# tensorboy/centerpose

Hardware: AMD Instinct MI355X
Metric: images/sec end-to-end (backbone+decode), DLA-34 512x512 (higher is better)
Workload: dtype f32

## Files before the change

### centerpose_amd/csrc/head_wino24.hip

```cpp
#include "igemm.h"

#define HW_THREADS 512
#define HW_PH 18
#define HW_PW 18
#define HW_PWP 20
#define HW_C 64
#define HW_CGS (HW_C / 4)
#define HW_CG (HW_PH * HW_PWP * 4)
#define HW_PATCH (HW_CGS * HW_CG)
#define HW_F4 (HW_PH * HW_PW * HW_CGS)
#define HW_SLOTS ((HW_F4 + HW_THREADS - 1) / HW_THREADS)
#define HW_LDR 36
#define HW_RED (16 * 32 * HW_LDR)
#define HW_LDM 36
#define HW_MID (256 * HW_LDM)
#define HW_SMEM_FLOATS (2 * HW_RED)
#define HW_SMEM_FLOATS_MM (HW_RED + HW_MID > HW_PATCH ? HW_RED + HW_MID : HW_PATCH)

typedef float hw_v2 __attribute__((ext_vector_type(2)));
typedef float hw_v4 __attribute__((ext_vector_type(4)));

struct HwHead {
    const float* w2;
    const float* b2;
    float* out2;
    int n2, ld2, act2;
};
struct HwGrid {
    int tilesX, tilesY;
    unsigned mTx, mTy;
};
__device__ __forceinline__ hw_v4 hw_lds4(const float* p) { return *reinterpret_cast<const hw_v4*>(p); }
__device__ __forceinline__ int hw_div(int n, int d, unsigned magic) { return d == 1 ? n : (int)__umulhi((unsigned)n, magic); }

__device__ __forceinline__ void hw_write_share(const f32x16 (&acc)[3], const int vh, const int P, float* wq)
{
#pragma unroll
    for (int j = 0; j < 4; ++j) {
        hw_v4 q[3];
#pragma unroll
        for (int nu = 0; nu < 3; ++nu) q[nu] = (hw_v4){acc[nu][4 * j], acc[nu][4 * j + 1], acc[nu][4 * j + 2], acc[nu][4 * j + 3]};
        hw_v4 c0, c1;
        if (vh == 0) {
            const hw_v4 s1 = q[1] + q[2], d1 = q[1] - q[2];
            c0 = P == 0 ? q[0] + s1 : s1;
            c1 = d1;
        } else {
            const hw_v4 s2 = q[0] + q[1], d2 = q[0] - q[1];
            c0 = P == 0 ? s2 : 4.f * s2;
            c1 = P == 0 ? 2.f * d2 : 8.f * d2 + q[2];
        }
        *reinterpret_cast<hw_v4*>(wq + 8 * j) = c0;
        *reinterpret_cast<hw_v4*>(wq + 32 * HW_LDR + 8 * j) = c1;
    }
}

template <int N2, int MM, bool STAG>
__global__ __launch_bounds__(HW_THREADS, 1) void head_wino24_kernel(const ConvArgs a, const HwGrid gd, const HwHead hd)
{
    static_assert(!(STAG && MM), "the second-MFMA-phase form has no staggered variant");
    extern __shared__ __attribute__((aligned(16))) float smem[];
    const int tid = threadIdx.x, lane = tid & 63, wv = __builtin_amdgcn_readfirstlane(tid >> 6);
    const int xi = wv & 3, vh = wv >> 2;
    const int h = lane >> 5, m = lane & 31;
    const int NTILES = (a.Cout + 31) >> 5;
    int t_ = ig_xcd_remap(blockIdx.x, gridDim.x), q_;
    q_ = hw_div(t_, gd.tilesX, gd.mTx); const int tx = t_ - q_ * gd.tilesX; t_ = q_;
    q_ = hw_div(t_, gd.tilesY, gd.mTy); const int ty = t_ - q_ * gd.tilesY;
    const int b = q_;
    const int y0 = ty * 16, x0 = tx * 16;
    const int ld = a.srcLd[0];
    const float* __restrict__ x = a.src[0];

    {
        float4 rg[HW_SLOTS];
        int lo[HW_SLOTS];
        bool ok[HW_SLOTS];
#pragma unroll
        for (int s = 0; s < HW_SLOTS; ++s) {
            const int idx = tid + s * HW_THREADS;
            const int pp = idx / HW_CGS, q = idx % HW_CGS;
            const int py = pp / HW_PW, px = pp - py * HW_PW;
            const int gy = y0 - 1 + py, gx = x0 - 1 + px;
            const bool inl = idx < HW_F4;
            ok[s] = inl && gy >= 0 && gy < a.H && gx >= 0 && gx < a.W;
            const int go = ok[s] ? ((b * a.H + gy) * a.W + gx) * ld + q * 4 : 0;
            lo[s] = inl ? ((q * HW_PH + py) * HW_PWP + (px ^ ((py >> 1) & 3))) * 4 : -1;
            rg[s] = ig_ldg4(x + go);
        }
#pragma unroll
        for (int s = 0; s < HW_SLOTS; ++s)
            if (lo[s] >= 0) {
                float4 v = rg[s];
                if (!ok[s]) v = make_float4(0.f, 0.f, 0.f, 0.f);
                *reinterpret_cast<float4*>(smem + lo[s]) = v;
            }
    }
    const float* up = a.w + ((size_t)xi * NTILES * (HW_C / 8)) * 1536 + (size_t)(3 * vh) * 256 + lane * 4;
    const int nlin = NTILES * (HW_C / 8);
    float4 bq[2][3];
#pragma unroll
    for (int nu = 0; nu < 3; ++nu) bq[0][nu] = ig_ldg4(up + nu * 256);
    __syncthreads();
    if constexpr (STAG) {
        if (vh == 1) __syncthreads();
    }

    const int rA = xi == 0 ? 0 : (xi == 2 ? 2 : 1);
    const int rB = xi == 2 ? 1 : (xi == 3 ? 3 : 2);
    const float sg1 = xi == 1 ? 1.f : -1.f;
    const hw_v2 sg = {sg1, sg1};
    const int tyy = m >> 2, txx = m & 3;
    const int sA = (tyy + (rA >> 1)) & 3, sB = (tyy + (rB >> 1)) & 3;
    const int baseA = ((2 * tyy + rA) * HW_PWP + 4 * txx) * 4 + h * HW_CG;
    const int baseB = ((2 * tyy + rB) * HW_PWP + 4 * txx) * 4 + h * HW_CG;
    int offA[4], offB[4];
#pragma unroll
    for (int jj = 0; jj < 4; ++jj) { offA[jj] = baseA + ((jj ^ sA) << 2); offB[jj] = baseB + ((jj ^ sB) << 2); }
    hw_v2 vl[HW_C / 8][3], vhh[HW_C / 8][3];
#pragma unroll
    for (int kc = 0; kc < HW_C / 8; ++kc) {
        const float* pc = smem + kc * 2 * HW_CG;
        hw_v2 tl[5], th[5];
        if (vh == 0) {
#pragma unroll
            for (int j = 0; j < 5; ++j) {
                const hw_v4 da = hw_lds4(pc + offA[j & 3] + (j >> 2) * 16), db = hw_lds4(pc + offB[j & 3] + (j >> 2) * 16);
                tl[j] = __builtin_elementwise_fma(sg, db.xy, da.xy);
                th[j] = __builtin_elementwise_fma(sg, db.zw, da.zw);
            }
        } else {
#pragma unroll
            for (int j = 0; j < 5; ++j) {
                const int jc = j + 1;
                const hw_v4 da = hw_lds4(pc + offA[jc & 3] + (jc >> 2) * 16), db = hw_lds4(pc + offB[jc & 3] + (jc >> 2) * 16);
                tl[j] = __builtin_elementwise_fma(sg, db.xy, da.xy);
                th[j] = __builtin_elementwise_fma(sg, db.zw, da.zw);
            }
        }
        const hw_v2 k4 = {4.f, 4.f}, kn4 = {-4.f, -4.f}, k2 = {2.f, 2.f}, kn2 = {-2.f, -2.f};
        if (vh == 0) {
            const hw_v2 al = __builtin_elementwise_fma(kn4, tl[2], tl[4]), ah = __builtin_elementwise_fma(kn4, th[2], th[4]);
            const hw_v2 bl = __builtin_elementwise_fma(kn4, tl[1], tl[3]), bh = __builtin_elementwise_fma(kn4, th[1], th[3]);
            vl[kc][0] = __builtin_elementwise_fma(k4, tl[0] - tl[2], tl[4] - tl[2]); vhh[kc][0] = __builtin_elementwise_fma(k4, th[0] - th[2], th[4] - th[2]);
            vl[kc][1] = al + bl; vhh[kc][1] = ah + bh;
            vl[kc][2] = al - bl; vhh[kc][2] = ah - bh;
        } else {
            const hw_v2 cl = tl[3] - tl[1], ch = th[3] - th[1];
            const hw_v2 fl = tl[2] - tl[0], fh = th[2] - th[0];
            vl[kc][0] = __builtin_elementwise_fma(k2, fl, cl); vhh[kc][0] = __builtin_elementwise_fma(k2, fh, ch);
            vl[kc][1] = __builtin_elementwise_fma(kn2, fl, cl); vhh[kc][1] = __builtin_elementwise_fma(kn2, fh, ch);
            vl[kc][2] = __builtin_elementwise_fma(kn4, fl, tl[4] - tl[2]); vhh[kc][2] = __builtin_elementwise_fma(kn4, fh, th[4] - th[2]);
        }
#pragma unroll
        for (int nu = 0; nu < 3; ++nu) asm volatile("" : "+v"(vl[kc][nu]), "+v"(vhh[kc][nu]));
        __builtin_amdgcn_sched_barrier(0);
    }
    if constexpr (STAG) {
        if (vh == 0) __syncthreads();
    } else {
        __syncthreads();
    }

    float acc2[2][2][N2 > 0 ? N2 : 1];
#pragma unroll
    for (int i = 0; i < 2; ++i)
#pragma unroll
        for (int k = 0; k < 2; ++k)
#pragma unroll
            for (int j = 0; j < (N2 > 0 ? N2 : 1); ++j) acc2[i][k][j] = 0.f;
    f32x16 acc2m;
#pragma unroll
    for (int r = 0; r < 16; ++r) acc2m[r] = 0.f;
    constexpr int J0 = MM ? 32 : 0;
    float* const mid = smem + HW_RED;
    const int n4 = tid & 7, bb = (tid >> 3) & 1, mi = tid >> 4;
    const int ity = mi >> 2, itx = mi & 3;
    const int itrd = (bb * 32 + mi) * HW_LDR + n4 * 4;
    const int wpo = (wv * 64 + m) * HW_LDR + 4 * h;

    int lin = 0;
    if constexpr (!MM) {
        hw_v4 sc = {0.f, 0.f, 0.f, 0.f}, sh = sc, w2r[N2];
#pragma unroll
        for (int j = 0; j < N2; ++j) w2r[j] = sc;
        hw_v4 rq[8];
        auto red_read = [&](int P) __attribute__((always_inline)) {
            int rbase = itrd + P * HW_RED;
            asm volatile("" : "+v"(rbase));
            const float* rp = smem + rbase;
#pragma unroll
            for (int w = 0; w < 8; ++w) rq[w] = hw_lds4(rp + w * 64 * HW_LDR);
        };
        auto red_sum = [&](int P) __attribute__((always_inline)) {
            const hw_v4 r0 = rq[0] + rq[4], r1 = rq[1] + rq[5], r2 = rq[2] + rq[6], r3 = rq[3] + rq[7];
            hw_v4 yv[2];
            yv[0] = (r0 + r1) + r2;
            yv[1] = (r1 - r2) - r3;
#pragma unroll
            for (int aa = 0; aa < 2; ++aa) {
                hw_v4 v = __builtin_elementwise_fma(yv[aa], sc, sh);
                v = (hw_v4){cp_relu(v.x), cp_relu(v.y), cp_relu(v.z), cp_relu(v.w)};
#pragma unroll
                for (int j = 0; j < N2; ++j) {
                    const hw_v4 w = w2r[j];
                    acc2[P][aa][j] = fmaf(v.w, w.w, fmaf(v.z, w.z, fmaf(v.y, w.y, fmaf(v.x, w.x, acc2[P][aa][j]))));
                }
            }
        };
        if constexpr (STAG) {
            auto chunk = [&](const int kc, f32x16 (&acc)[3], auto&& ride) __attribute__((always_inline)) {
                ++lin;
                const float* un = up + (size_t)(lin < nlin ? lin : nlin - 1) * 1536;
                __builtin_amdgcn_sched_barrier(0);
#pragma unroll
                for (int nu = 0; nu < 3; ++nu) {
                    if (nu == 1) {
#pragma unroll
                        for (int q = 0; q < 3; ++q) bq[(kc + 1) & 1][q] = ig_ldg4(un + q * 256);
                        __builtin_amdgcn_sched_barrier(0);
                    }
                    if (nu == 2) {
                        ride();
                        __builtin_amdgcn_sched_barrier(0);
                    }
                    const float4 bbv = bq[kc & 1][nu];
                    acc[nu] = __builtin_amdgcn_mfma_f32_32x32x2f32(bbv.x, vl[kc][nu].x, acc[nu], 0, 0, 0);
                    acc[nu] = __builtin_amdgcn_mfma_f32_32x32x2f32(bbv.y, vl[kc][nu].y, acc[nu], 0, 0, 0);
                    acc[nu] = __builtin_amdgcn_mfma_f32_32x32x2f32(bbv.z, vhh[kc][nu].x, acc[nu], 0, 0, 0);
                    acc[nu] = __builtin_amdgcn_mfma_f32_32x32x2f32(bbv.w, vhh[kc][nu].y, acc[nu], 0, 0, 0);
                }
                __builtin_amdgcn_sched_barrier(0);
            };
            auto tile_end = [&](const int nt, const f32x16 (&acc)[3], const bool barrier_first) __attribute__((always_inline)) {
                const int ncol = nt * 32 + n4 * 4;
                sc = *reinterpret_cast<const hw_v4*>(a.scale + ncol);
                sh = *reinterpret_cast<const hw_v4*>(a.shift + ncol);
#pragma unroll
                for (int j = 0; j < N2; ++j) w2r[j] = *reinterpret_cast<const hw_v4*>(hd.w2 + (size_t)j * hd.ld2 + ncol);
                if (barrier_first) __syncthreads();
#pragma unroll
                for (int P = 0; P < 2; ++P) {
                    int wbase = wpo + P * HW_RED;
                    asm volatile("" : "+v"(wbase));
                    hw_write_share(acc, vh, P, smem + wbase);
                }
            };
            const auto nothing = [] {};
            if (vh == 0) {
#pragma unroll 1
                for (int nt = 0; nt < NTILES; ++nt) {
                    const bool prev = nt > 0;
                    f32x16 acc[3];
#pragma unroll
                    for (int nu = 0; nu < 3; ++nu)
#pragma unroll
                        for (int r = 0; r < 16; ++r) acc[nu][r] = 0.f;
#pragma unroll
                    for (int kc = 0; kc < 5; ++kc) chunk(kc, acc, nothing);
                    __syncthreads();
                    chunk(5, acc, [&] { if (prev) red_read(0); });
                    chunk(6, acc, [&] { if (prev) { red_sum(0); red_read(1); } });
                    chunk(7, acc, [&] { if (prev) red_sum(1); });
                    tile_end(nt, acc, true);
                }
            } else {
#pragma unroll 1
                for (int nt = 0; nt < NTILES; ++nt) {
                    const bool prev = nt > 0;
                    f32x16 acc[3];
#pragma unroll
                    for (int nu = 0; nu < 3; ++nu)
#pragma unroll
                        for (int r = 0; r < 16; ++r) acc[nu][r] = 0.f;
                    __syncthreads();
                    chunk(0, acc, [&] { if (prev) red_read(0); });
                    chunk(1, acc, [&] { if (prev) red_sum(0); });
                    chunk(2, acc, [&] { if (prev) red_read(1); });
                    chunk(3, acc, [&] { if (prev) red_sum(1); });
                    __syncthreads();
#pragma unroll
                    for (int kc = 4; kc < 8; ++kc) chunk(kc, acc, nothing);
                    tile_end(nt, acc, false);
                }
            }
            __syncthreads();
        } else {
#pragma unroll 1
        for (int nt = 0; nt < NTILES; ++nt) {
            const bool prev = nt > 0;
            f32x16 acc[3];
#pragma unroll
            for (int nu = 0; nu < 3; ++nu)
#pragma unroll
                for (int r = 0; r < 16; ++r) acc[nu][r] = 0.f;
#pragma unroll
            for (int kc = 0; kc < HW_C / 8; ++kc) {
                ++lin;
                const float* un = up + (size_t)(lin < nlin ? lin : nlin - 1) * 1536;
                __builtin_amdgcn_sched_barrier(0);
#pragma unroll
                for (int nu = 0; nu < 3; ++nu) {
                    if (nu == 1) {
#pragma unroll
                        for (int q = 0; q < 3; ++q) bq[(kc + 1) & 1][q] = ig_ldg4(un + q * 256);
                        __builtin_amdgcn_sched_barrier(0);
                    }
                    if (nu == 2 && prev) {
                        if (kc == 0) red_read(0);
                        if (kc == 2) red_sum(0);
                        if (kc == 4) red_read(1);
                        if (kc == 6) red_sum(1);
                        __builtin_amdgcn_sched_barrier(0);
                    }
                    const float4 bbv = bq[kc & 1][nu];
                    acc[nu] = __builtin_amdgcn_mfma_f32_32x32x2f32(bbv.x, vl[kc][nu].x, acc[nu], 0, 0, 0);
                    acc[nu] = __builtin_amdgcn_mfma_f32_32x32x2f32(bbv.y, vl[kc][nu].y, acc[nu], 0, 0, 0);
                    acc[nu] = __builtin_amdgcn_mfma_f32_32x32x2f32(bbv.z, vhh[kc][nu].x, acc[nu], 0, 0, 0);
                    acc[nu] = __builtin_amdgcn_mfma_f32_32x32x2f32(bbv.w, vhh[kc][nu].y, acc[nu], 0, 0, 0);
                }
                __builtin_amdgcn_sched_barrier(0);
            }
            const int ncol = nt * 32 + n4 * 4;
            sc = *reinterpret_cast<const hw_v4*>(a.scale + ncol);
            sh = *reinterpret_cast<const hw_v4*>(a.shift + ncol);
#pragma unroll
            for (int j = 0; j < N2; ++j) w2r[j] = *reinterpret_cast<const hw_v4*>(hd.w2 + (size_t)j * hd.ld2 + ncol);
            if (prev) __syncthreads();
#pragma unroll
            for (int P = 0; P < 2; ++P) {
                int wbase = wpo + P * HW_RED;
                asm volatile("" : "+v"(wbase));
                float* wq = smem + wbase;
#pragma unroll
                for (int j = 0; j < 4; ++j) {
                    hw_v4 q[3];
#pragma unroll
                    for (int nu = 0; nu < 3; ++nu) q[nu] = (hw_v4){acc[nu][4 * j], acc[nu][4 * j + 1], acc[nu][4 * j + 2], acc[nu][4 * j + 3]};
                    hw_v4 c0, c1;
                    if (vh == 0) {
                        const hw_v4 s1 = q[1] + q[2], d1 = q[1] - q[2];
                        c0 = P == 0 ? q[0] + s1 : s1;
                        c1 = d1;
                    } else {
                        const hw_v4 s2 = q[0] + q[1], d2 = q[0] - q[1];
                        c0 = P == 0 ? s2 : 4.f * s2;
                        c1 = P == 0 ? 2.f * d2 : 8.f * d2 + q[2];
                    }
                    *reinterpret_cast<hw_v4*>(wq + 8 * j) = c0;
                    *reinterpret_cast<hw_v4*>(wq + 32 * HW_LDR + 8 * j) = c1;
                }
            }
            __syncthreads();
        }
        }
        red_read(0); red_sum(0);
        red_read(1); red_sum(1);
    } else {
#pragma unroll 1
    for (int nt = 0; nt < NTILES; ++nt) {
        f32x16 acc[3];
#pragma unroll
        for (int nu = 0; nu < 3; ++nu)
#pragma unroll
            for (int r = 0; r < 16; ++r) acc[nu][r] = 0.f;
#pragma unroll
        for (int kc = 0; kc < HW_C / 8; ++kc) {
            ++lin;
            const float* un = up + (size_t)(lin < nlin ? lin : nlin - 1) * 1536;
            __builtin_amdgcn_sched_barrier(0);
#pragma unroll
            for (int nu = 0; nu < 3; ++nu) {
                if (nu == 1) {
#pragma unroll
                    for (int q = 0; q < 3; ++q) bq[(kc + 1) & 1][q] = ig_ldg4(un + q * 256);
                    __builtin_amdgcn_sched_barrier(0);
                }
                const float4 bbv = bq[kc & 1][nu];
                acc[nu] = __builtin_amdgcn_mfma_f32_32x32x2f32(bbv.x, vl[kc][nu].x, acc[nu], 0, 0, 0);
                acc[nu] = __builtin_amdgcn_mfma_f32_32x32x2f32(bbv.y, vl[kc][nu].y, acc[nu], 0, 0, 0);
                acc[nu] = __builtin_amdgcn_mfma_f32_32x32x2f32(bbv.z, vhh[kc][nu].x, acc[nu], 0, 0, 0);
                acc[nu] = __builtin_amdgcn_mfma_f32_32x32x2f32(bbv.w, vhh[kc][nu].y, acc[nu], 0, 0, 0);
            }
            __builtin_amdgcn_sched_barrier(0);
        }

        const int ncol = nt * 32 + n4 * 4;
        const hw_v4 sc = *reinterpret_cast<const hw_v4*>(a.scale + ncol), sh = *reinterpret_cast<const hw_v4*>(a.shift + ncol);
        hw_v4 w2r[N2 > 0 ? N2 : 1];
#pragma unroll
        for (int j = 0; j < N2; ++j) w2r[j] = *reinterpret_cast<const hw_v4*>(hd.w2 + (size_t)(J0 + j) * hd.ld2 + ncol);
        hw_v4 w2f[MM ? 4 : 1];
#pragma unroll
        for (int P = 0; P < 2; ++P) {
            if (MM && P == 1) __syncthreads();
            int wbase = wpo + (MM ? 0 : P * HW_RED), rbase = itrd + (MM ? 0 : P * HW_RED);
            asm volatile("" : "+v"(wbase), "+v"(rbase));
            float* wq = smem + wbase;
#pragma unroll
            for (int j = 0; j < 4; ++j) {
                hw_v4 q[3];
#pragma unroll
                for (int nu = 0; nu < 3; ++nu) q[nu] = (hw_v4){acc[nu][4 * j], acc[nu][4 * j + 1], acc[nu][4 * j + 2], acc[nu][4 * j + 3]};
                hw_v4 c0, c1;
                if (vh == 0) {
                    const hw_v4 s1 = q[1] + q[2], d1 = q[1] - q[2];
                    c0 = P == 0 ? q[0] + s1 : s1;
                    c1 = d1;
                } else {
                    const hw_v4 s2 = q[0] + q[1], d2 = q[0] - q[1];
                    c0 = P == 0 ? s2 : 4.f * s2;
                    c1 = P == 0 ? 2.f * d2 : 8.f * d2 + q[2];
                }
                *reinterpret_cast<hw_v4*>(wq + 8 * j) = c0;
                *reinterpret_cast<hw_v4*>(wq + 32 * HW_LDR + 8 * j) = c1;
            }
            if constexpr (MM) {
                if (P == 1) {
                    const int nmm = hd.n2 < 32 ? hd.n2 : 32;
                    const bool live = m < nmm;
                    const float* wrow = hd.w2 + (size_t)(live ? m : nmm - 1) * hd.ld2 + nt * 32 + 4 * h;
#pragma unroll
                    for (int s4 = 0; s4 < 4; ++s4) {
                        const float4 t4 = ig_ldg4(wrow + 8 * s4);
                        w2f[s4] = live ? (hw_v4){t4.x, t4.y, t4.z, t4.w} : (hw_v4){0.f, 0.f, 0.f, 0.f};
                    }
                }
            }
            __syncthreads();
            const float* rp = smem + rbase;
            hw_v4 r0 = hw_lds4(rp) + hw_lds4(rp + 4 * 64 * HW_LDR);
            const hw_v4 r1 = hw_lds4(rp + 64 * HW_LDR) + hw_lds4(rp + 5 * 64 * HW_LDR);
            const hw_v4 r2 = hw_lds4(rp + 2 * 64 * HW_LDR) + hw_lds4(rp + 6 * 64 * HW_LDR);
            const hw_v4 r3 = hw_lds4(rp + 3 * 64 * HW_LDR) + hw_lds4(rp + 7 * 64 * HW_LDR);
            hw_v4 yv[2];
            yv[0] = (r0 + r1) + r2;
            yv[1] = (r1 - r2) - r3;
#pragma unroll
            for (int aa = 0; aa < 2; ++aa) {
                hw_v4 v = __builtin_elementwise_fma(yv[aa], sc, sh);
                v = (hw_v4){cp_relu(v.x), cp_relu(v.y), cp_relu(v.z), cp_relu(v.w)};
#pragma unroll
                for (int j = 0; j < N2; ++j) {
                    const hw_v4 w = w2r[j];
                    acc2[P][aa][j] = fmaf(v.w, w.w, fmaf(v.z, w.z, fmaf(v.y, w.y, fmaf(v.x, w.x, acc2[P][aa][j]))));
                }
                if constexpr (MM) {
                    *reinterpret_cast<hw_v4*>(mid + ((2 * ity + aa) * 16 + 4 * itx + 2 * P + bb) * HW_LDM + n4 * 4) = v;
                }
            }
        }
        if constexpr (MM) {
            __syncthreads();
            const float* mp = mid + (32 * wv + m) * HW_LDM + 4 * h;
            hw_v4 mf[4];
#pragma unroll
            for (int s4 = 0; s4 < 4; ++s4) mf[s4] = hw_lds4(mp + 8 * s4);
#pragma unroll
            for (int s4 = 0; s4 < 4; ++s4) {
                acc2m = __builtin_amdgcn_mfma_f32_32x32x2f32(w2f[s4].x, mf[s4].x, acc2m, 0, 0, 0);
                acc2m = __builtin_amdgcn_mfma_f32_32x32x2f32(w2f[s4].y, mf[s4].y, acc2m, 0, 0, 0);
                acc2m = __builtin_amdgcn_mfma_f32_32x32x2f32(w2f[s4].z, mf[s4].z, acc2m, 0, 0, 0);
                acc2m = __builtin_amdgcn_mfma_f32_32x32x2f32(w2f[s4].w, mf[s4].w, acc2m, 0, 0, 0);
            }
            __syncthreads();
        }
    }

    }
    const size_t HW = (size_t)a.H * a.W;
    if constexpr (MM) {
        const int p = 32 * wv + m, ox = x0 + (p & 15), oy = y0 + (p >> 4);
        const int nmm = hd.n2 < 32 ? hd.n2 : 32;
        if (ox < a.W && oy < a.H) {
#pragma unroll
            for (int r = 0; r < 16; ++r) {
                const int j = (r & 3) + 8 * (r >> 2) + 4 * h;
                if (j < nmm) hd.out2[((size_t)b * hd.n2 + j) * HW + (size_t)oy * a.W + ox] = cp_act(acc2m[r] + hd.b2[j], hd.act2);
            }
        }
    }
    if constexpr (N2 > 0) {
#pragma unroll
        for (int P = 0; P < 2; ++P) {
            const int ox = x0 + 4 * itx + 2 * P + bb, oy = y0 + 2 * ity;
#pragma unroll
            for (int aa = 0; aa < 2; ++aa)
#pragma unroll
                for (int j = 0; j < N2; ++j) {
                    float v = acc2[P][aa][j];
                    v += __shfl_xor(v, 1);
                    v += __shfl_xor(v, 2);
                    v += __shfl_xor(v, 4);
                    if ((tid & 7) == 0 && J0 + j < hd.n2 && ox < a.W && oy + aa < a.H)
                        hd.out2[((size_t)b * hd.n2 + J0 + j) * HW + (size_t)(oy + aa) * a.W + ox] = cp_act(v + hd.b2[J0 + j], hd.act2);
                }
        }
    }
}

static unsigned hw_magic(int d) { return d <= 1 ? 0u : (unsigned)(((1ull << 32) + (unsigned)d - 1) / (unsigned)d); }

template <int N2, int MM, bool STAG = false>
static int launch_head_wino24(const ConvArgs& a, hipStream_t s, const HwHead& hd)
{
    const int smem = (MM ? HW_SMEM_FLOATS_MM : HW_SMEM_FLOATS) * 4;
    static CpLdsGuard guard;
    {
        const hipError_t e = guard.ensure((const void*)head_wino24_kernel<N2, MM, STAG>, smem);
        if (e != hipSuccess) { cp_set_error("head_wino24: cannot reserve %d B LDS: %s", smem, hipGetErrorString(e)); return 2; }
    }
    HwGrid gd;
    gd.tilesX = cp_cdiv(a.W, 16); gd.tilesY = cp_cdiv(a.H, 16);
    gd.mTx = hw_magic(gd.tilesX); gd.mTy = hw_magic(gd.tilesY);
    const long long grid = (long long)a.B * gd.tilesX * gd.tilesY;
    const long long dmax = gd.tilesX > gd.tilesY ? gd.tilesX : gd.tilesY;
    if (grid * dmax >= (1ll << 32)) { cp_set_error("head_wino24: grid %lld too large", grid); return 1; }
    hipLaunchKernelGGL((head_wino24_kernel<N2, MM, STAG>), dim3((unsigned)grid), dim3(HW_THREADS), smem, s, a, gd, hd);
    cp_note_kernel("head_wino24_kernel<%d, %d>", N2, MM);
    return 0;
}

int cp_launch_head3x3_1x1_w24(const ConvArgs& a, const float* w2, const float* b2, float* out2, int n2, int ld2, int act2, hipStream_t s)
{
    const bool ok = a.nsrc == 1 && a.kh == 3 && a.kw == 3 && a.sy == 1 && a.sx == 1 && a.py == 1 && a.px == 1 && a.Ho == a.H &&
                    a.Wo == a.W && a.srcC[0] == 64 && a.srcLd[0] % 4 == 0 && a.Cout % 32 == 0 && a.act == CP_ACT_RELU && !a.res &&
                    n2 >= 1 && n2 <= 34 && ld2 % 4 == 0 && ld2 >= a.Cout &&
                    (((size_t)a.src[0] | (size_t)a.w | (size_t)w2 | (size_t)a.scale | (size_t)a.shift) & 15) == 0 &&
                    (long long)a.B * a.H * a.W * a.srcLd[0] < (1ll << 31);
    if (!ok) return -1;
    HwHead hd;
    hd.w2 = w2; hd.b2 = b2; hd.out2 = out2; hd.n2 = n2; hd.ld2 = ld2; hd.act2 = act2;
    const char* sw = getenv("CP_HEAD_STAGGER");
    const bool stag = !(sw && sw[0] == '0');
    if (n2 == 1) return stag ? launch_head_wino24<1, 0, true>(a, s, hd) : launch_head_wino24<1, 0>(a, s, hd);
    if (n2 == 2) return stag ? launch_head_wino24<2, 0, true>(a, s, hd) : launch_head_wino24<2, 0>(a, s, hd);
    if (n2 <= 32) return launch_head_wino24<0, 1>(a, s, hd);
    if (n2 == 33) return launch_head_wino24<1, 1>(a, s, hd);
    return launch_head_wino24<2, 1>(a, s, hd);
}
```

Measured before the change: 2232.

## Make head Winograd kernel persistent with next-tile patch prefetch overlapped with MFMA

The head 3x3+1x1 Winograd kernel becomes a persistent loop over tiles. Each block computes the next tile's coordinates and issues its global patch loads during the current tile's MFMA phase, so the input fetch for tile n+1 overlaps compute for tile n. The grid is capped at the CU count only when CP_HEAD_PERSIST or CP_HEAD_BLOCKS is set, and the default trait is false. By default the grid still equals the tile count, so each block runs one iteration of the new loop structure and keeps the extra register pressure.

```diff
diff --git a/centerpose_amd/csrc/head_wino24.hip b/centerpose_amd/csrc/head_wino24.hip
--- a/centerpose_amd/csrc/head_wino24.hip
+++ b/centerpose_amd/csrc/head_wino24.hip
@@ -27,11 +27,17 @@
     int n2, ld2, act2;
 };
 struct HwGrid {
-    int tilesX, tilesY;
+    int tilesX, tilesY, tiles;
     unsigned mTx, mTy;
 };
+template <bool V> struct HwFlag { static constexpr bool value = V; };
 __device__ __forceinline__ hw_v4 hw_lds4(const float* p) { return *reinterpret_cast<const hw_v4*>(p); }
 __device__ __forceinline__ int hw_div(int n, int d, unsigned magic) { return d == 1 ? n : (int)__umulhi((unsigned)n, magic); }
+
+template <int K> __device__ __forceinline__ float hw_xor_lane(float v)
+{
+    return __int_as_float(__builtin_amdgcn_ds_swizzle(__float_as_int(v), (K << 10) | 0x1f));
+}
 
 __device__ __forceinline__ void hw_write_share(const f32x16 (&acc)[3], const int vh, const int P, float* wq)
 {
@@ -62,178 +68,226 @@
     extern __shared__ __attribute__((aligned(16))) float smem[];
     const int tid = threadIdx.x, lane = tid & 63, wv = __builtin_amdgcn_readfirstlane(tid >> 6);
     const int xi = wv & 3, vh = wv >> 2;
-    const int h = lane >> 5, m = lane & 31;
     const int NTILES = (a.Cout + 31) >> 5;
-    int t_ = ig_xcd_remap(blockIdx.x, gridDim.x), q_;
-    q_ = hw_div(t_, gd.tilesX, gd.mTx); const int tx = t_ - q_ * gd.tilesX; t_ = q_;
-    q_ = hw_div(t_, gd.tilesY, gd.mTy); const int ty = t_ - q_ * gd.tilesY;
-    const int b = q_;
-    const int y0 = ty * 16, x0 = tx * 16;
     const int ld = a.srcLd[0];
     const float* __restrict__ x = a.src[0];
-
-    {
-        float4 rg[HW_SLOTS];
-        int lo[HW_SLOTS];
-        bool ok[HW_SLOTS];
+    const int tiles = gd.tiles;
+
+    auto tile_at = [&](const int vv, int& b_, int& y0_, int& x0_) __attribute__((always_inline)) {
+        int t_ = ig_xcd_remap(vv, tiles), q_;
+        q_ = hw_div(t_, gd.tilesX, gd.mTx); x0_ = (t_ - q_ * gd.tilesX) * 16; t_ = q_;
+        q_ = hw_div(t_, gd.tilesY, gd.mTy); y0_ = (t_ - q_ * gd.tilesY) * 16;
+        b_ = q_;
+    };
+    float4 rg[HW_SLOTS];
+    unsigned okm;
+    auto patch_issue = [&](const int b_, const int y0_, const int x0_) __attribute__((always_inline)) {
+        int t = tid;
+        asm volatile("" : "+v"(t));
+        const int q = t & (HW_CGS - 1), pp0 = t >> 4;
+        okm = 0u;
 #pragma unroll
         for (int s = 0; s < HW_SLOTS; ++s) {
-            const int idx = tid + s * HW_THREADS;
-            const int pp = idx / HW_CGS, q = idx % HW_CGS;
+            const int pp = pp0 + s * (HW_THREADS / HW_CGS);
             const int py = pp / HW_PW, px = pp - py * HW_PW;
-            const int gy = y0 - 1 + py, gx = x0 - 1 + px;
-            const bool inl = idx < HW_F4;
-            ok[s] = inl && gy >= 0 && gy < a.H && gx >= 0 && gx < a.W;
-            const int go = ok[s] ? ((b * a.H + gy) * a.W + gx) * ld + q * 4 : 0;
-            lo[s] = inl ? ((q * HW_PH + py) * HW_PWP + (px ^ ((py >> 1) & 3))) * 4 : -1;
+            const int gy = y0_ - 1 + py, gx = x0_ - 1 + px;
+            const bool inl = (s + 1) * HW_THREADS <= HW_F4 || t + s * HW_THREADS < HW_F4;
+            const bool ok = inl && gy >= 0 && gy < a.H && gx >= 0 && gx < a.W;
+            const int go = ok ? ((b_ * a.H + gy) * a.W + gx) * ld + q * 4 : 0;
+            okm |= ok ? (1u << s) : 0u;
             rg[s] = ig_ldg4(x + go);
         }
-#pragma unroll
-        for (int s = 0; s < HW_SLOTS; ++s)
-            if (lo[s] >= 0) {
+    };
+    auto patch_store = [&]() __attribute__((always_inline)) {
+        int t = tid;
+        asm volatile("" : "+v"(t));
+        const int q = t & (HW_CGS - 1), pp0 = t >> 4;
+#pragma unroll
+        for (int s = 0; s < HW_SLOTS; ++s) {
+            const int pp = pp0 + s * (HW_THREADS / HW_CGS);
+            const int py = pp / HW_PW, px = pp - py * HW_PW;
+            if ((s + 1) * HW_THREADS <= HW_F4 || t + s * HW_THREADS < HW_F4) {
                 float4 v = rg[s];
-                if (!ok[s]) v = make_float4(0.f, 0.f, 0.f, 0.f);
-                *reinterpret_cast<float4*>(smem + lo[s]) = v;
-            }
-    }
-    const float* up = a.w + ((size_t)xi * NTILES * (HW_C / 8)) * 1536 + (size_t)(3 * vh) * 256 + lane * 4;
+                if (!((okm >> s) & 1u)) v = make_float4(0.f, 0.f, 0.f, 0.f);
+                *reinterpret_cast<float4*>(smem + ((q * HW_PH + py) * HW_PWP + (px ^ ((py >> 1) & 3))) * 4) = v;
+            }
+        }
+    };
+
+    int v = blockIdx.x, b, y0, x0;
+    tile_at(v, b, y0, x0);
+    patch_issue(b, y0, x0);
+    const float* up = a.w + ((size_t)xi * NTILES * (HW_C / 8)) * 1536 + (size_t)(3 * vh) * 256;
     const int nlin = NTILES * (HW_C / 8);
     float4 bq[2][3];
 #pragma unroll
-    for (int nu = 0; nu < 3; ++nu) bq[0][nu] = ig_ldg4(up + nu * 256);
-    __syncthreads();
-    if constexpr (STAG) {
-        if (vh == 1) __syncthreads();
-    }
+    for (int nu = 0; nu < 3; ++nu) bq[0][nu] = ig_ldg4(up + nu * 256 + (unsigned)lane * 4);
+    int lin = 0;
 
     const int rA = xi == 0 ? 0 : (xi == 2 ? 2 : 1);
     const int rB = xi == 2 ? 1 : (xi == 3 ? 3 : 2);
-    const float sg1 = xi == 1 ? 1.f : -1.f;
-    const hw_v2 sg = {sg1, sg1};
-    const int tyy = m >> 2, txx = m & 3;
-    const int sA = (tyy + (rA >> 1)) & 3, sB = (tyy + (rB >> 1)) & 3;
-    const int baseA = ((2 * tyy + rA) * HW_PWP + 4 * txx) * 4 + h * HW_CG;
-    const int baseB = ((2 * tyy + rB) * HW_PWP + 4 * txx) * 4 + h * HW_CG;
-    int offA[4], offB[4];
-#pragma unroll
-    for (int jj = 0; jj < 4; ++jj) { offA[jj] = baseA + ((jj ^ sA) << 2); offB[jj] = baseB + ((jj ^ sB) << 2); }
-    hw_v2 vl[HW_C / 8][3], vhh[HW_C / 8][3];
-#pragma unroll
-    for (int kc = 0; kc < HW_C / 8; ++kc) {
-        const float* pc = smem + kc * 2 * HW_CG;
-        hw_v2 tl[5], th[5];
-        if (vh == 0) {
-#pragma unroll
-            for (int j = 0; j < 5; ++j) {
-                const hw_v4 da = hw_lds4(pc + offA[j & 3] + (j >> 2) * 16), db = hw_lds4(pc + offB[j & 3] + (j >> 2) * 16);
-                tl[j] = __builtin_elementwise_fma(sg, db.xy, da.xy);
-                th[j] = __builtin_elementwise_fma(sg, db.zw, da.zw);
-            }
-        } else {
-#pragma unroll
-            for (int j = 0; j < 5; ++j) {
-                const int jc = j + 1;
-                const hw_v4 da = hw_lds4(pc + offA[jc & 3] + (jc >> 2) * 16), db = hw_lds4(pc + offB[jc & 3] + (jc >> 2) * 16);
-                tl[j] = __builtin_elementwise_fma(sg, db.xy, da.xy);
-                th[j] = __builtin_elementwise_fma(sg, db.zw, da.zw);
-            }
-        }
-        const hw_v2 k4 = {4.f, 4.f}, kn4 = {-4.f, -4.f}, k2 = {2.f, 2.f}, kn2 = {-2.f, -2.f};
-        if (vh == 0) {
-            const hw_v2 al = __builtin_elementwise_fma(kn4, tl[2], tl[4]), ah = __builtin_elementwise_fma(kn4, th[2], th[4]);
-            const hw_v2 bl = __builtin_elementwise_fma(kn4, tl[1], tl[3]), bh = __builtin_elementwise_fma(kn4, th[1], th[3]);
-            vl[kc][0] = __builtin_elementwise_fma(k4, tl[0] - tl[2], tl[4] - tl[2]); vhh[kc][0] = __builtin_elementwise_fma(k4, th[0] - th[2], th[4] - th[2]);
-            vl[kc][1] = al + bl; vhh[kc][1] = ah + bh;
-            vl[kc][2] = al - bl; vhh[kc][2] = ah - bh;
-        } else {
-            const hw_v2 cl = tl[3] - tl[1], ch = th[3] - th[1];
-            const hw_v2 fl = tl[2] - tl[0], fh = th[2] - th[0];
-            vl[kc][0] = __builtin_elementwise_fma(k2, fl, cl); vhh[kc][0] = __builtin_elementwise_fma(k2, fh, ch);
-            vl[kc][1] = __builtin_elementwise_fma(kn2, fl, cl); vhh[kc][1] = __builtin_elementwise_fma(kn2, fh, ch);
-            vl[kc][2] = __builtin_elementwise_fma(kn4, fl, tl[4] - tl[2]); vhh[kc][2] = __builtin_elementwise_fma(kn4, fh, th[4] - th[2]);
-        }
-#pragma unroll
-        for (int nu = 0; nu < 3; ++nu) asm volatile("" : "+v"(vl[kc][nu]), "+v"(vhh[kc][nu]));
-        __builtin_amdgcn_sched_barrier(0);
-    }
-    if constexpr (STAG) {
-        if (vh == 0) __syncthreads();
-    } else {
-        __syncthreads();
-    }
-
-    float acc2[2][2][N2 > 0 ? N2 : 1];
-#pragma unroll
-    for (int i = 0; i < 2; ++i)
-#pragma unroll
-        for (int k = 0; k < 2; ++k)
-#pragma unroll
-            for (int j = 0; j < (N2 > 0 ? N2 : 1); ++j) acc2[i][k][j] = 0.f;
-    f32x16 acc2m;
-#pragma unroll
-    for (int r = 0; r < 16; ++r) acc2m[r] = 0.f;
     constexpr int J0 = MM ? 32 : 0;
     float* const mid = smem + HW_RED;
-    const int n4 = tid & 7, bb = (tid >> 3) & 1, mi = tid >> 4;
-    const int ity = mi >> 2, itx = mi & 3;
-    const int itrd = (bb * 32 + mi) * HW_LDR + n4 * 4;
-    const int wpo = (wv * 64 + m) * HW_LDR + 4 * h;
-
-    int lin = 0;
-    if constexpr (!MM) {
-        hw_v4 sc = {0.f, 0.f, 0.f, 0.f}, sh = sc, w2r[N2];
-#pragma unroll
-        for (int j = 0; j < N2; ++j) w2r[j] = sc;
-        hw_v4 rq[8];
-        auto red_read = [&](int P) __attribute__((always_inline)) {
-            int rbase = itrd + P * HW_RED;
-            asm volatile("" : "+v"(rbase));
-            const float* rp = smem + rbase;
-#pragma unroll
-            for (int w = 0; w < 8; ++w) rq[w] = hw_lds4(rp + w * 64 * HW_LDR);
+    const size_t HW = (size_t)a.H * a.W;
+    float b2r[N2 > 0 ? N2 : 1];
+#pragma unroll
+    for (int j = 0; j < N2; ++j) b2r[j] = *(const __attribute__((address_space(4))) float*)(hd.b2 + J0 + j);
+
+#pragma unroll 1
+    for (;;) {
+        const int vn = v + (int)gridDim.x;
+        const bool more = vn < tiles;
+        int nb, ny0, nx0;
+        tile_at(more ? vn : v, nb, ny0, nx0);
+
+        patch_store();
+        __syncthreads();
+        if constexpr (STAG) {
+            if (vh == 1) __syncthreads();
+        }
+
+        int lv = tid & 63;
+        float sg1 = xi == 1 ? 1.f : -1.f;
+        asm volatile("" : "+v"(lv), "+v"(sg1));
+        const hw_v2 sg = {sg1, sg1};
+        const int tyy = (lv & 31) >> 2, txx = lv & 3;
+        const int sA = (tyy + (rA >> 1)) & 3, sB = (tyy + (rB >> 1)) & 3;
+        const int baseA = ((2 * tyy + rA) * HW_PWP + 4 * txx) * 4 + (lv >> 5) * HW_CG;
+        const int baseB = ((2 * tyy + rB) * HW_PWP + 4 * txx) * 4 + (lv >> 5) * HW_CG;
+        int offA[4], offB[4];
+#pragma unroll
+        for (int jj = 0; jj < 4; ++jj) { offA[jj] = baseA + ((jj ^ sA) << 2); offB[jj] = baseB + ((jj ^ sB) << 2); }
+        hw_v2 vl[HW_C / 8][3], vhh[HW_C / 8][3];
+#pragma unroll
+        for (int kc = 0; kc < HW_C / 8; ++kc) {
+            const float* pc = smem + kc * 2 * HW_CG;
+            hw_v2 tl[5], th[5];
+            if (vh == 0) {
+#pragma unroll
+                for (int j = 0; j < 5; ++j) {
+                    const hw_v4 da = hw_lds4(pc + offA[j & 3] + (j >> 2) * 16), db = hw_lds4(pc + offB[j & 3] + (j >> 2) * 16);
+                    tl[j] = __builtin_elementwise_fma(sg, db.xy, da.xy);
+                    th[j] = __builtin_elementwise_fma(sg, db.zw, da.zw);
+                }
+            } else {
+#pragma unroll
+                for (int j = 0; j < 5; ++j) {
+                    const int jc = j + 1;
+                    const hw_v4 da = hw_lds4(pc + offA[jc & 3] + (jc >> 2) * 16), db = hw_lds4(pc + offB[jc & 3] + (jc >> 2) * 16);
+                    tl[j] = __builtin_elementwise_fma(sg, db.xy, da.xy);
+                    th[j] = __builtin_elementwise_fma(sg, db.zw, da.zw);
+                }
+            }
+            const hw_v2 k4 = {4.f, 4.f}, kn4 = {-4.f, -4.f}, k2 = {2.f, 2.f}, kn2 = {-2.f, -2.f};
+            if (vh == 0) {
+                const hw_v2 al = __builtin_elementwise_fma(kn4, tl[2], tl[4]), ah = __builtin_elementwise_fma(kn4, th[2], th[4]);
+                const hw_v2 bl = __builtin_elementwise_fma(kn4, tl[1], tl[3]), bh = __builtin_elementwise_fma(kn4, th[1], th[3]);
+                vl[kc][0] = __builtin_elementwise_fma(k4, tl[0] - tl[2], tl[4] - tl[2]); vhh[kc][0] = __builtin_elementwise_fma(k4, th[0] - th[2], th[4] - th[2]);
+                vl[kc][1] = al + bl; vhh[kc][1] = ah + bh;
+                vl[kc][2] = al - bl; vhh[kc][2] = ah - bh;
+            } else {
+                const hw_v2 cl = tl[3] - tl[1], ch = th[3] - th[1];
+                const hw_v2 fl = tl[2] - tl[0], fh = th[2] - th[0];
+                vl[kc][0] = __builtin_elementwise_fma(k2, fl, cl); vhh[kc][0] = __builtin_elementwise_fma(k2, fh, ch);
+                vl[kc][1] = __builtin_elementwise_fma(kn2, fl, cl); vhh[kc][1] = __builtin_elementwise_fma(kn2, fh, ch);
+                vl[kc][2] = __builtin_elementwise_fma(kn4, fl, tl[4] - tl[2]); vhh[kc][2] = __builtin_elementwise_fma(kn4, fh, th[4] - th[2]);
+            }
+#pragma unroll
+            for (int nu = 0; nu < 3; ++nu) asm volatile("" : "+v"(vl[kc][nu]), "+v"(vhh[kc][nu]));
+            __builtin_amdgcn_sched_barrier(0);
+        }
+        if constexpr (STAG) {
+            if (vh == 0) __syncthreads();
+        } else {
+            __syncthreads();
+        }
+
+        float acc2[2][2][N2 > 0 ? N2 : 1];
+#pragma unroll
+        for (int i = 0; i < 2; ++i)
+#pragma unroll
+            for (int k = 0; k < 2; ++k)
+#pragma unroll
+                for (int j = 0; j < (N2 > 0 ? N2 : 1); ++j) acc2[i][k][j] = 0.f;
+        f32x16 acc2m;
+#pragma unroll
+        for (int r = 0; r < 16; ++r) acc2m[r] = 0.f;
+
+        auto chunk = [&](const int kc, f32x16 (&acc)[3], auto&& ride) __attribute__((always_inline)) {
+            lin = lin + 1 < nlin ? lin + 1 : 0;
+            const float* un = up + (size_t)lin * 1536;
+            int tc = tid;
+            asm volatile("" : "+v"(tc));
+            const unsigned ul = (tc & 63) * 4;
+            __builtin_amdgcn_sched_barrier(0);
+#pragma unroll
+            for (int nu = 0; nu < 3; ++nu) {
+                if (nu == 1) {
+#pragma unroll
+                    for (int q = 0; q < 3; ++q) bq[(kc + 1) & 1][q] = ig_ldg4(un + q * 256 + ul);
+                    __builtin_amdgcn_sched_barrier(0);
+                }
+                if (nu == 2) {
+                    ride();
+                    __builtin_amdgcn_sched_barrier(0);
+                }
+                const float4 bbv = bq[kc & 1][nu];
+                acc[nu] = __builtin_amdgcn_mfma_f32_32x32x2f32(bbv.x, vl[kc][nu].x, acc[nu], 0, 0, 0);
+                acc[nu] = __builtin_amdgcn_mfma_f32_32x32x2f32(bbv.y, vl[kc][nu].y, acc[nu], 0, 0, 0);
+                acc[nu] = __builtin_amdgcn_mfma_f32_32x32x2f32(bbv.z, vhh[kc][nu].x, acc[nu], 0, 0, 0);
+                acc[nu] = __builtin_amdgcn_mfma_f32_32x32x2f32(bbv.w, vhh[kc][nu].y, acc[nu], 0, 0, 0);
+            }
+            __builtin_amdgcn_sched_barrier(0);
         };
-        auto red_sum = [&](int P) __attribute__((always_inline)) {
-            const hw_v4 r0 = rq[0] + rq[4], r1 = rq[1] + rq[5], r2 = rq[2] + rq[6], r3 = rq[3] + rq[7];
-            hw_v4 yv[2];
-            yv[0] = (r0 + r1) + r2;
-            yv[1] = (r1 - r2) - r3;
-#pragma unroll
-            for (int aa = 0; aa < 2; ++aa) {
-                hw_v4 v = __builtin_elementwise_fma(yv[aa], sc, sh);
-                v = (hw_v4){cp_relu(v.x), cp_relu(v.y), cp_relu(v.z), cp_relu(v.w)};
-#pragma unroll
-                for (int j = 0; j < N2; ++j) {
-                    const hw_v4 w = w2r[j];
-                    acc2[P][aa][j] = fmaf(v.w, w.w, fmaf(v.z, w.z, fmaf(v.y, w.y, fmaf(v.x, w.x, acc2[P][aa][j]))));
-                }
-            }
+        auto request_next = [&]() __attribute__((always_inline)) {
+            if (more) {
+                patch_issue(nb, ny0, nx0);
+            } else {
+                okm = 0u;
+#pragma unroll
+                for (int s = 0; s < HW_SLOTS; ++s) rg[s] = make_float4(0.f, 0.f, 0.f, 0.f);
+            }
+            __builtin_amdgcn_sched_barrier(0);
         };
-        if constexpr (STAG) {
-            auto chunk = [&](const int kc, f32x16 (&acc)[3], auto&& ride) __attribute__((always_inline)) {
-                ++lin;
-                const float* un = up + (size_t)(lin < nlin ? lin : nlin - 1) * 1536;
-                __builtin_amdgcn_sched_barrier(0);
-#pragma unroll
-                for (int nu = 0; nu < 3; ++nu) {
-                    if (nu == 1) {
-#pragma unroll
-                        for (int q = 0; q < 3; ++q) bq[(kc + 1) & 1][q] = ig_ldg4(un + q * 256);
-                        __builtin_amdgcn_sched_barrier(0);
+        const auto nothing = [] {};
+
+        if constexpr (!MM) {
+            hw_v4 sc = {0.f, 0.f, 0.f, 0.f}, sh = sc, w2r[N2];
+#pragma unroll
+            for (int j = 0; j < N2; ++j) w2r[j] = sc;
+            hw_v4 rq[8];
+#pragma unroll
+            for (int w = 0; w < 8; ++w) rq[w] = sc;
+            auto red_read = [&](int P) __attribute__((always_inline)) {
+                int tr = tid;
+                asm volatile("" : "+v"(tr));
+                int rbase = (((tr >> 3) & 1) * 32 + (tr >> 4)) * HW_LDR + (tr & 7) * 4 + P * HW_RED;
+                asm volatile("" : "+v"(rbase));
+                const float* rp = smem + rbase;
+#pragma unroll
+                for (int w = 0; w < 8; ++w) rq[w] = hw_lds4(rp + w * 64 * HW_LDR);
+            };
+            auto red_sum = [&](int P) __attribute__((always_inline)) {
+                const hw_v4 r0 = rq[0] + rq[4], r1 = rq[1] + rq[5], r2 = rq[2] + rq[6], r3 = rq[3] + rq[7];
+                hw_v4 yv[2];
+                yv[0] = (r0 + r1) + r2;
+                yv[1] = (r1 - r2) - r3;
+#pragma unroll
+                for (int aa = 0; aa < 2; ++aa) {
+                    hw_v4 v = __builtin_elementwise_fma(yv[aa], sc, sh);
+                    v = (hw_v4){cp_relu(v.x), cp_relu(v.y), cp_relu(v.z), cp_relu(v.w)};
+#pragma unroll
+                    for (int j = 0; j < N2; ++j) {
+                        const hw_v4 w = w2r[j];
+                        acc2[P][aa][j] = fmaf(v.w, w.w, fmaf(v.z, w.z, fmaf(v.y, w.y, fmaf(v.x, w.x, acc2[P][aa][j]))));
                     }
-                    if (nu == 2) {
-                        ride();
-                        __builtin_amdgcn_sched_barrier(0);
-                    }
-                    const float4 bbv = bq[kc & 1][nu];
-                    acc[nu] = __builtin_amdgcn_mfma_f32_32x32x2f32(bbv.x, vl[kc][nu].x, acc[nu], 0, 0, 0);
-                    acc[nu] = __builtin_amdgcn_mfma_f32_32x32x2f32(bbv.y, vl[kc][nu].y, acc[nu], 0, 0, 0);
-                    acc[nu] = __builtin_amdgcn_mfma_f32_32x32x2f32(bbv.z, vhh[kc][nu].x, acc[nu], 0, 0, 0);
-                    acc[nu] = __builtin_amdgcn_mfma_f32_32x32x2f32(bbv.w, vhh[kc][nu].y, acc[nu], 0, 0, 0);
-                }
-                __builtin_amdgcn_sched_barrier(0);
+                }
             };
             auto tile_end = [&](const int nt, const f32x16 (&acc)[3], const bool barrier_first) __attribute__((always_inline)) {
-                const int ncol = nt * 32 + n4 * 4;
+                int nq = tid;
+                asm volatile("" : "+v"(nq));
+                nq &= 7;
+                const int ncol = nt * 32 + nq * 4;
                 sc = *reinterpret_cast<const hw_v4*>(a.scale + ncol);
                 sh = *reinterpret_cast<const hw_v4*>(a.shift + ncol);
 #pragma unroll
@@ -241,38 +295,37 @@
                 if (barrier_first) __syncthreads();
 #pragma unroll
                 for (int P = 0; P < 2; ++P) {
-                    int wbase = wpo + P * HW_RED;
+                    int tw = tid;
+                    asm volatile("" : "+v"(tw));
+                    int wbase = ((tw >> 6) * 64 + (tw & 31)) * HW_LDR + 4 * ((tw >> 5) & 1) + P * HW_RED;
                     asm volatile("" : "+v"(wbase));
                     hw_write_share(acc, vh, P, smem + wbase);
                 }
             };
-            const auto nothing = [] {};
-            if (vh == 0) {
-#pragma unroll 1
-                for (int nt = 0; nt < NTILES; ++nt) {
+            auto zero = [&](f32x16 (&acc)[3]) __attribute__((always_inline)) {
+#pragma unroll
+                for (int nu = 0; nu < 3; ++nu)
+#pragma unroll
+                    for (int r = 0; r < 16; ++r) acc[nu][r] = 0.f;
+            };
+            if constexpr (STAG) {
+                auto tileA = [&](const int nt, auto last) __attribute__((always_inline)) {
                     const bool prev = nt > 0;
                     f32x16 acc[3];
-#pragma unroll
-                    for (int nu = 0; nu < 3; ++nu)
-#pragma unroll
-                        for (int r = 0; r < 16; ++r) acc[nu][r] = 0.f;
+                    zero(acc);
 #pragma unroll
                     for (int kc = 0; kc < 5; ++kc) chunk(kc, acc, nothing);
                     __syncthreads();
                     chunk(5, acc, [&] { if (prev) red_read(0); });
                     chunk(6, acc, [&] { if (prev) { red_sum(0); red_read(1); } });
                     chunk(7, acc, [&] { if (prev) red_sum(1); });
+                    if constexpr (decltype(last)::value) request_next();
                     tile_end(nt, acc, true);
-                }
-            } else {
-#pragma unroll 1
-                for (int nt = 0; nt < NTILES; ++nt) {
+                };
+                auto tileB = [&](const int nt, auto last) __attribute__((always_inline)) {
                     const bool prev = nt > 0;
                     f32x16 acc[3];
-#pragma unroll
-                    for (int nu = 0; nu < 3; ++nu)
-#pragma unroll
-                        for (int r = 0; r < 16; ++r) acc[nu][r] = 0.f;
+                    zero(acc);
                     __syncthreads();
                     chunk(0, acc, [&] { if (prev) red_read(0); });
                     chunk(1, acc, [&] { if (prev) red_sum(0); });
@@ -281,225 +334,157 @@
                     __syncthreads();
 #pragma unroll
                     for (int kc = 4; kc < 8; ++kc) chunk(kc, acc, nothing);
+                    if constexpr (decltype(last)::value) request_next();
                     tile_end(nt, acc, false);
-                }
-            }
-            __syncthreads();
+                };
+                if (vh == 0) {
+#pragma unroll 1
+                    for (int nt = 0; nt < NTILES - 1; ++nt) tileA(nt, HwFlag<false>());
+                    tileA(NTILES - 1, HwFlag<true>());
+                } else {
+#pragma unroll 1
+                    for (int nt = 0; nt < NTILES - 1; ++nt) tileB(nt, HwFlag<false>());
+                    tileB(NTILES - 1, HwFlag<true>());
+                }
+                __syncthreads();
+            } else {
+                auto tileL = [&](const int nt, auto last) __attribute__((always_inline)) {
+                    const bool prev = nt > 0;
+                    f32x16 acc[3];
+                    zero(acc);
+                    chunk(0, acc, [&] { if (prev) red_read(0); });
+                    chunk(1, acc, nothing);
+                    chunk(2, acc, [&] { if (prev) red_sum(0); });
+                    chunk(3, acc, nothing);
+                    chunk(4, acc, [&] { if (prev) red_read(1); });
+                    chunk(5, acc, nothing);
+                    chunk(6, acc, [&] { if (prev) red_sum(1); });
+                    chunk(7, acc, nothing);
+                    if constexpr (decltype(last)::value) request_next();
+                    tile_end(nt, acc, prev);
+                    __syncthreads();
+                };
+#pragma unroll 1
+                for (int nt = 0; nt < NTILES - 1; ++nt) tileL(nt, HwFlag<false>());
+                tileL(NTILES - 1, HwFlag<true>());
+            }
+            red_read(0); red_sum(0);
+            red_read(1); red_sum(1);
         } else {
+            auto tileM = [&](const int nt, auto last) __attribute__((always_inline)) {
+                f32x16 acc[3];
+#pragma unroll
+                for (int nu = 0; nu < 3; ++nu)
+#pragma unroll
+                    for (int r = 0; r < 16; ++r) acc[nu][r] = 0.f;
+#pragma unroll
+                for (int kc = 0; kc < HW_C / 8; ++kc) chunk(kc, acc, nothing);
+                if constexpr (decltype(last)::value) request_next();
+
+                int te = tid;
+                asm volatile("" : "+v"(te));
+                const int nq = te & 7, eb = (te >> 3) & 1, emi = te >> 4, em = te & 31, eh = (te >> 5) & 1;
+                const int ncol = nt * 32 + nq * 4;
+                const hw_v4 sc = *reinterpret_cast<const hw_v4*>(a.scale + ncol), sh = *reinterpret_cast<const hw_v4*>(a.shift + ncol);
+                hw_v4 w2r[N2 > 0 ? N2 : 1];
+#pragma unroll
+                for (int j = 0; j < N2; ++j) w2r[j] = *reinterpret_cast<const hw_v4*>(hd.w2 + (size_t)(J0 + j) * hd.ld2 + ncol);
+                hw_v4 w2f[4];
+#pragma unroll
+                for (int P = 0; P < 2; ++P) {
+                    if (P == 1) __syncthreads();
+                    int wbase = ((te >> 6) * 64 + em) * HW_LDR + 4 * eh, rbase = (eb * 32 + emi) * HW_LDR + nq * 4;
+                    asm volatile("" : "+v"(wbase), "+v"(rbase));
+                    hw_write_share(acc, vh, P, smem + wbase);
+                    if (P == 1) {
+                        const int nmm = hd.n2 < 32 ? hd.n2 : 32;
+                        const bool live = em < nmm;
+                        const float* wrow = hd.w2 + (size_t)(live ? em : nmm - 1) * hd.ld2 + nt * 32 + 4 * eh;
+#pragma unroll
+                        for (int s4 = 0; s4 < 4; ++s4) {
+                            const float4 t4 = ig_ldg4(wrow + 8 * s4);
+                            w2f[s4] = live ? (hw_v4){t4.x, t4.y, t4.z, t4.w} : (hw_v4){0.f, 0.f, 0.f, 0.f};
+                        }
+                    }
+                    __syncthreads();
+                    const float* rp = smem + rbase;
+                    hw_v4 r0 = hw_lds4(rp) + hw_lds4(rp + 4 * 64 * HW_LDR);
+                    const hw_v4 r1 = hw_lds4(rp + 64 * HW_LDR) + hw_lds4(rp + 5 * 64 * HW_LDR);
+                    const hw_v4 r2 = hw_lds4(rp + 2 * 64 * HW_LDR) + hw_lds4(rp + 6 * 64 * HW_LDR);
+                    const hw_v4 r3 = hw_lds4(rp + 3 * 64 * HW_LDR) + hw_lds4(rp + 7 * 64 * HW_LDR);
+                    hw_v4 yv[2];
+                    yv[0] = (r0 + r1) + r2;
+                    yv[1] = (r1 - r2) - r3;
+#pragma unroll
+                    for (int aa = 0; aa < 2; ++aa) {
+                        hw_v4 v = __builtin_elementwise_fma(yv[aa], sc, sh);
+                        v = (hw_v4){cp_relu(v.x), cp_relu(v.y), cp_relu(v.z), cp_relu(v.w)};
+#pragma unroll
+                        for (int j = 0; j < N2; ++j) {
+                            const hw_v4 w = w2r[j];
+                            acc2[P][aa][j] = fmaf(v.w, w.w, fmaf(v.z, w.z, fmaf(v.y, w.y, fmaf(v.x, w.x, acc2[P][aa][j]))));
+                        }
+                        *reinterpret_cast<hw_v4*>(mid + ((2 * (emi >> 2) + aa) * 16 + 4 * (emi & 3) + 2 * P + eb) * HW_LDM + nq * 4) = v;
+                    }
+                }
+                __syncthreads();
+                const float* mp = mid + (32 * wv + em) * HW_LDM + 4 * eh;
+                hw_v4 mf[4];
+#pragma unroll
+                for (int s4 = 0; s4 < 4; ++s4) mf[s4] = hw_lds4(mp + 8 * s4);
+#pragma unroll
+                for (int s4 = 0; s4 < 4; ++s4) {
+                    acc2m = __builtin_amdgcn_mfma_f32_32x32x2f32(w2f[s4].x, mf[s4].x, acc2m, 0, 0, 0);
+                    acc2m = __builtin_amdgcn_mfma_f32_32x32x2f32(w2f[s4].y, mf[s4].y, acc2m, 0, 0, 0);
+                    acc2m = __builtin_amdgcn_mfma_f32_32x32x2f32(w2f[s4].z, mf[s4].z, acc2m, 0, 0, 0);
+                    acc2m = __builtin_amdgcn_mfma_f32_32x32x2f32(w2f[s4].w, mf[s4].w, acc2m, 0, 0, 0);
+                }
+                __syncthreads();
+            };
 #pragma unroll 1
-        for (int nt = 0; nt < NTILES; ++nt) {
-            const bool prev = nt > 0;
-            f32x16 acc[3];
-#pragma unroll
-            for (int nu = 0; nu < 3; ++nu)
-#pragma unroll
-                for (int r = 0; r < 16; ++r) acc[nu][r] = 0.f;
-#pragma unroll
-            for (int kc = 0; kc < HW_C / 8; ++kc) {
-                ++lin;
-                const float* un = up + (size_t)(lin < nlin ? lin : nlin - 1) * 1536;
-                __builtin_amdgcn_sched_barrier(0);
-#pragma unroll
-                for (int nu = 0; nu < 3; ++nu) {
-                    if (nu == 1) {
-#pragma unroll
-                        for (int q = 0; q < 3; ++q) bq[(kc + 1) & 1][q] = ig_ldg4(un + q * 256);
-                        __builtin_amdgcn_sched_barrier(0);
+            for (int nt = 0; nt < NTILES - 1; ++nt) tileM(nt, HwFlag<false>());
+            tileM(NTILES - 1, HwFlag<true>());
+        }
+
+        int to = tid;
+        asm volatile("" : "+v"(to));
+        if constexpr (MM) {
+            const int p = 32 * wv + (to & 31), ox = x0 + (p & 15), oy = y0 + (p >> 4);
+            const int nmm = hd.n2 < 32 ? hd.n2 : 32;
+            if (ox < a.W && oy < a.H) {
+#pragma unroll
+                for (int r = 0; r < 16; ++r) {
+                    const int j = (r & 3) + 8 * (r >> 2) + 4 * ((to >> 5) & 1);
+                    if (j < nmm) hd.out2[((size_t)b * hd.n2 + j) * HW + (size_t)oy * a.W + ox] = cp_act(acc2m[r] + hd.b2[j], hd.act2);
+                }
+            }
+        }
+        if constexpr (N2 > 0) {
+#pragma unroll
+            for (int P = 0; P < 2; ++P) {
+                const int ox = x0 + 4 * ((to >> 4) & 3) + 2 * P + ((to >> 3) & 1), oy = y0 + 2 * (to >> 6);
+#pragma unroll
+                for (int aa = 0; aa < 2; ++aa)
+#pragma unroll
+                    for (int j = 0; j < N2; ++j) {
+                        float v = acc2[P][aa][j];
+                        v += hw_xor_lane<1>(v);
+                        v += hw_xor_lane<2>(v);
+                        v += hw_xor_lane<4>(v);
+                        if ((to & 7) == 0 && J0 + j < hd.n2 && ox < a.W && oy + aa < a.H)
+                            hd.out2[((size_t)b * hd.n2 + J0 + j) * HW + (size_t)(oy + aa) * a.W + ox] = cp_act(v + b2r[j], hd.act2);
                     }
-                    if (nu == 2 && prev) {
-                        if (kc == 0) red_read(0);
-                        if (kc == 2) red_sum(0);
-                        if (kc == 4) red_read(1);
-                        if (kc == 6) red_sum(1);
-                        __builtin_amdgcn_sched_barrier(0);
-                    }
-                    const float4 bbv = bq[kc & 1][nu];
-                    acc[nu] = __builtin_amdgcn_mfma_f32_32x32x2f32(bbv.x, vl[kc][nu].x, acc[nu], 0, 0, 0);
-                    acc[nu] = __builtin_amdgcn_mfma_f32_32x32x2f32(bbv.y, vl[kc][nu].y, acc[nu], 0, 0, 0);
-                    acc[nu] = __builtin_amdgcn_mfma_f32_32x32x2f32(bbv.z, vhh[kc][nu].x, acc[nu], 0, 0, 0);
-                    acc[nu] = __builtin_amdgcn_mfma_f32_32x32x2f32(bbv.w, vhh[kc][nu].y, acc[nu], 0, 0, 0);
-                }
-                __builtin_amdgcn_sched_barrier(0);
-            }
-            const int ncol = nt * 32 + n4 * 4;
-            sc = *reinterpret_cast<const hw_v4*>(a.scale + ncol);
-            sh = *reinterpret_cast<const hw_v4*>(a.shift + ncol);
-#pragma unroll
-            for (int j = 0; j < N2; ++j) w2r[j] = *reinterpret_cast<const hw_v4*>(hd.w2 + (size_t)j * hd.ld2 + ncol);
-            if (prev) __syncthreads();
-#pragma unroll
-            for (int P = 0; P < 2; ++P) {
-                int wbase = wpo + P * HW_RED;
-                asm volatile("" : "+v"(wbase));
-                float* wq = smem + wbase;
-#pragma unroll
-                for (int j = 0; j < 4; ++j) {
-                    hw_v4 q[3];
-#pragma unroll
-                    for (int nu = 0; nu < 3; ++nu) q[nu] = (hw_v4){acc[nu][4 * j], acc[nu][4 * j + 1], acc[nu][4 * j + 2], acc[nu][4 * j + 3]};
-                    hw_v4 c0, c1;
-                    if (vh == 0) {
-                        const hw_v4 s1 = q[1] + q[2], d1 = q[1] - q[2];
-                        c0 = P == 0 ? q[0] + s1 : s1;
-                        c1 = d1;
-                    } else {
-                        const hw_v4 s2 = q[0] + q[1], d2 = q[0] - q[1];
-                        c0 = P == 0 ? s2 : 4.f * s2;
-                        c1 = P == 0 ? 2.f * d2 : 8.f * d2 + q[2];
-                    }
-                    *reinterpret_cast<hw_v4*>(wq + 8 * j) = c0;
-                    *reinterpret_cast<hw_v4*>(wq + 32 * HW_LDR + 8 * j) = c1;
-                }
-            }
-            __syncthreads();
-        }
-        }
-        red_read(0); red_sum(0);
-        red_read(1); red_sum(1);
-    } else {
-#pragma unroll 1
-    for (int nt = 0; nt < NTILES; ++nt) {
-        f32x16 acc[3];
-#pragma unroll
-        for (int nu = 0; nu < 3; ++nu)
-#pragma unroll
-            for (int r = 0; r < 16; ++r) acc[nu][r] = 0.f;
-#pragma unroll
-        for (int kc = 0; kc < HW_C / 8; ++kc) {
-            ++lin;
-            const float* un = up + (size_t)(lin < nlin ? lin : nlin - 1) * 1536;
-            __builtin_amdgcn_sched_barrier(0);
-#pragma unroll
-            for (int nu = 0; nu < 3; ++nu) {
-                if (nu == 1) {
-#pragma unroll
-                    for (int q = 0; q < 3; ++q) bq[(kc + 1) & 1][q] = ig_ldg4(un + q * 256);
-                    __builtin_amdgcn_sched_barrier(0);
-                }
-                const float4 bbv = bq[kc & 1][nu];
-                acc[nu] = __builtin_amdgcn_mfma_f32_32x32x2f32(bbv.x, vl[kc][nu].x, acc[nu], 0, 0, 0);
-                acc[nu] = __builtin_amdgcn_mfma_f32_32x32x2f32(bbv.y, vl[kc][nu].y, acc[nu], 0, 0, 0);
-                acc[nu] = __builtin_amdgcn_mfma_f32_32x32x2f32(bbv.z, vhh[kc][nu].x, acc[nu], 0, 0, 0);
-                acc[nu] = __builtin_amdgcn_mfma_f32_32x32x2f32(bbv.w, vhh[kc][nu].y, acc[nu], 0, 0, 0);
-            }
-            __builtin_amdgcn_sched_barrier(0);
-        }
-
-        const int ncol = nt * 32 + n4 * 4;
-        const hw_v4 sc = *reinterpret_cast<const hw_v4*>(a.scale + ncol), sh = *reinterpret_cast<const hw_v4*>(a.shift + ncol);
-        hw_v4 w2r[N2 > 0 ? N2 : 1];
-#pragma unroll
-        for (int j = 0; j < N2; ++j) w2r[j] = *reinterpret_cast<const hw_v4*>(hd.w2 + (size_t)(J0 + j) * hd.ld2 + ncol);
-        hw_v4 w2f[MM ? 4 : 1];
-#pragma unroll
-        for (int P = 0; P < 2; ++P) {
-            if (MM && P == 1) __syncthreads();
-            int wbase = wpo + (MM ? 0 : P * HW_RED), rbase = itrd + (MM ? 0 : P * HW_RED);
-            asm volatile("" : "+v"(wbase), "+v"(rbase));
-            float* wq = smem + wbase;
-#pragma unroll
-            for (int j = 0; j < 4; ++j) {
-                hw_v4 q[3];
-#pragma unroll
-                for (int nu = 0; nu < 3; ++nu) q[nu] = (hw_v4){acc[nu][4 * j], acc[nu][4 * j + 1], acc[nu][4 * j + 2], acc[nu][4 * j + 3]};
-                hw_v4 c0, c1;
-                if (vh == 0) {
-                    const hw_v4 s1 = q[1] + q[2], d1 = q[1] - q[2];
-                    c0 = P == 0 ? q[0] + s1 : s1;
-                    c1 = d1;
-                } else {
-                    const hw_v4 s2 = q[0] + q[1], d2 = q[0] - q[1];
-                    c0 = P == 0 ? s2 : 4.f * s2;
-                    c1 = P == 0 ? 2.f * d2 : 8.f * d2 + q[2];
-                }
-                *reinterpret_cast<hw_v4*>(wq + 8 * j) = c0;
-                *reinterpret_cast<hw_v4*>(wq + 32 * HW_LDR + 8 * j) = c1;
-            }
-            if constexpr (MM) {
-                if (P == 1) {
-                    const int nmm = hd.n2 < 32 ? hd.n2 : 32;
-                    const bool live = m < nmm;
-                    const float* wrow = hd.w2 + (size_t)(live ? m : nmm - 1) * hd.ld2 + nt * 32 + 4 * h;
-#pragma unroll
-                    for (int s4 = 0; s4 < 4; ++s4) {
-                        const float4 t4 = ig_ldg4(wrow + 8 * s4);
-                        w2f[s4] = live ? (hw_v4){t4.x, t4.y, t4.z, t4.w} : (hw_v4){0.f, 0.f, 0.f, 0.f};
-                    }
-                }
-            }
-            __syncthreads();
-            const float* rp = smem + rbase;
-            hw_v4 r0 = hw_lds4(rp) + hw_lds4(rp + 4 * 64 * HW_LDR);
-            const hw_v4 r1 = hw_lds4(rp + 64 * HW_LDR) + hw_lds4(rp + 5 * 64 * HW_LDR);
-            const hw_v4 r2 = hw_lds4(rp + 2 * 64 * HW_LDR) + hw_lds4(rp + 6 * 64 * HW_LDR);
-            const hw_v4 r3 = hw_lds4(rp + 3 * 64 * HW_LDR) + hw_lds4(rp + 7 * 64 * HW_LDR);
-            hw_v4 yv[2];
-            yv[0] = (r0 + r1) + r2;
-            yv[1] = (r1 - r2) - r3;
-#pragma unroll
-            for (int aa = 0; aa < 2; ++aa) {
-                hw_v4 v = __builtin_elementwise_fma(yv[aa], sc, sh);
-                v = (hw_v4){cp_relu(v.x), cp_relu(v.y), cp_relu(v.z), cp_relu(v.w)};
-#pragma unroll
-                for (int j = 0; j < N2; ++j) {
-                    const hw_v4 w = w2r[j];
-                    acc2[P][aa][j] = fmaf(v.w, w.w, fmaf(v.z, w.z, fmaf(v.y, w.y, fmaf(v.x, w.x, acc2[P][aa][j]))));
-                }
-                if constexpr (MM) {
-                    *reinterpret_cast<hw_v4*>(mid + ((2 * ity + aa) * 16 + 4 * itx + 2 * P + bb) * HW_LDM + n4 * 4) = v;
-                }
-            }
-        }
-        if constexpr (MM) {
-            __syncthreads();
-            const float* mp = mid + (32 * wv + m) * HW_LDM + 4 * h;
-            hw_v4 mf[4];
-#pragma unroll
-            for (int s4 = 0; s4 < 4; ++s4) mf[s4] = hw_lds4(mp + 8 * s4);
-#pragma unroll
-            for (int s4 = 0; s4 < 4; ++s4) {
-                acc2m = __builtin_amdgcn_mfma_f32_32x32x2f32(w2f[s4].x, mf[s4].x, acc2m, 0, 0, 0);
-                acc2m = __builtin_amdgcn_mfma_f32_32x32x2f32(w2f[s4].y, mf[s4].y, acc2m, 0, 0, 0);
-                acc2m = __builtin_amdgcn_mfma_f32_32x32x2f32(w2f[s4].z, mf[s4].z, acc2m, 0, 0, 0);
-                acc2m = __builtin_amdgcn_mfma_f32_32x32x2f32(w2f[s4].w, mf[s4].w, acc2m, 0, 0, 0);
-            }
-            __syncthreads();
-        }
-    }
-
-    }
-    const size_t HW = (size_t)a.H * a.W;
-    if constexpr (MM) {
-        const int p = 32 * wv + m, ox = x0 + (p & 15), oy = y0 + (p >> 4);
-        const int nmm = hd.n2 < 32 ? hd.n2 : 32;
-        if (ox < a.W && oy < a.H) {
-#pragma unroll
-            for (int r = 0; r < 16; ++r) {
-                const int j = (r & 3) + 8 * (r >> 2) + 4 * h;
-                if (j < nmm) hd.out2[((size_t)b * hd.n2 + j) * HW + (size_t)oy * a.W + ox] = cp_act(acc2m[r] + hd.b2[j], hd.act2);
-            }
-        }
-    }
-    if constexpr (N2 > 0) {
-#pragma unroll
-        for (int P = 0; P < 2; ++P) {
-            const int ox = x0 + 4 * itx + 2 * P + bb, oy = y0 + 2 * ity;
-#pragma unroll
-            for (int aa = 0; aa < 2; ++aa)
-#pragma unroll
-                for (int j = 0; j < N2; ++j) {
-                    float v = acc2[P][aa][j];
-                    v += __shfl_xor(v, 1);
-                    v += __shfl_xor(v, 2);
-                    v += __shfl_xor(v, 4);
-                    if ((tid & 7) == 0 && J0 + j < hd.n2 && ox < a.W && oy + aa < a.H)
-                        hd.out2[((size_t)b * hd.n2 + J0 + j) * HW + (size_t)(oy + aa) * a.W + ox] = cp_act(v + hd.b2[J0 + j], hd.act2);
-                }
-        }
+            }
+        }
+        if (!more) break;
+        v = vn; b = nb; y0 = ny0; x0 = nx0;
+        __syncthreads();
     }
 }
 
 static unsigned hw_magic(int d) { return d <= 1 ? 0u : (unsigned)(((1ull << 32) + (unsigned)d - 1) / (unsigned)d); }
+
+template <int N2, int MM> struct HwPersistDefault { static constexpr bool value = false; };
 
 template <int N2, int MM, bool STAG = false>
 static int launch_head_wino24(const ConvArgs& a, hipStream_t s, const HwHead& hd)
@@ -513,9 +498,20 @@
     HwGrid gd;
     gd.tilesX = cp_cdiv(a.W, 16); gd.tilesY = cp_cdiv(a.H, 16);
     gd.mTx = hw_magic(gd.tilesX); gd.mTy = hw_magic(gd.tilesY);
-    const long long grid = (long long)a.B * gd.tilesX * gd.tilesY;
+    const long long tiles = (long long)a.B * gd.tilesX * gd.tilesY;
     const long long dmax = gd.tilesX > gd.tilesY ? gd.tilesX : gd.tilesY;
-    if (grid * dmax >= (1ll << 32)) { cp_set_error("head_wino24: grid %lld too large", grid); return 1; }
+    if (tiles * dmax >= (1ll << 32) || tiles >= (1ll << 30)) { cp_set_error("head_wino24: grid %lld too large", tiles); return 1; }
+    gd.tiles = (int)tiles;
+    const char* pw = getenv("CP_HEAD_PERSIST");
+    const char* cap = getenv("CP_HEAD_BLOCKS");
+    const long long ncap = cap ? atoll(cap) : 0;
+    const bool persist = pw && pw[0] ? pw[0] != '0' : (HwPersistDefault<N2, MM>::value || ncap >= 1);
+    long long grid = tiles;
+    if (persist) {
+        const int cus = cp_num_cus();
+        if (grid > cus) grid = cus;
+        if (ncap >= 1 && grid > ncap) grid = ncap;
+    }
     hipLaunchKernelGGL((head_wino24_kernel<N2, MM, STAG>), dim3((unsigned)grid), dim3(HW_THREADS), smem, s, a, gd, hd);
     cp_note_kernel("head_wino24_kernel<%d, %d>", N2, MM);
     return 0;
```

After: 2245, median of 4. Within noise of the previous version (+0.6%).
